# keurfonluu/stochopy

Hardware: AMD Instinct MI355X
Metric: objective-fn evals/sec (higher is better)
Workload: dtype f64; 1 GPU; de_rosenbrock_n128_p4096; method=de, objective=rosenbrock, dim=128, popsize_per_gpu=4096, popsize_total=4096, rng=philox, exchange=none

## Files before the change

include/stochopy_hip.h:

```cpp
#ifndef STOCHOPY_HIP_H
#define STOCHOPY_HIP_H

#include <stdint.h>

#ifdef __cplusplus
extern "C" {
#endif

#define SX_ABI_VERSION 1

enum {
    SX_FUN_ACKLEY = 0,
    SX_FUN_GRIEWANK = 1,
    SX_FUN_QUARTIC = 2,
    SX_FUN_RASTRIGIN = 3,
    SX_FUN_ROSENBROCK = 4,
    SX_FUN_SPHERE = 5,
    SX_FUN_STYBLINSKI_TANG = 6,
    SX_FUN_COUNT = 7
};

enum { SX_DE_RAND1BIN = 0, SX_DE_RAND2BIN = 1, SX_DE_BEST1BIN = 2, SX_DE_BEST2BIN = 3 };

enum {
    SX_RNG_HOST = 0,
    SX_RNG_PHILOX = 1
};

#define SX_STATUS_NONE 100

int sx_abi_version(void);
const char *sx_last_error(void);
int sx_device_count(void);
int sx_struct_size(int which);

int sx_sum_plan(int64_t m, int32_t *out, int cap);
int64_t sx_fun_terms(int fun_id, int n);

int64_t sx_num_partials(int64_t P, int n);
int sx_rows_per_workgroup(int n);
int sx_wide_from(void);
int64_t sx_de_num_partials(int64_t P, int n, int wide_from);
int sx_eval(int fun_id, const double *X, int64_t P, int n, int64_t ldx, const double *xm, const double *xstd,
            double *f, double *part_f, int64_t *part_i, void *stream);

int sx_philox_lhs(double *X, int64_t rows, int n, int64_t ld, int64_t row0, int64_t P, const double *lower,
                  const double *upper, uint32_t key0, uint32_t key1, void *stream);

int sx_argmin(const double *f, int64_t P, double *ws_f, int64_t *ws_i, int64_t ws_len, int64_t *out_idx,
              double *out_val, void *stream);

typedef struct sx_state {
    int64_t it;
    int64_t gbidx;
    double gfit;
    double dx;
    int32_t status;
    int32_t done;
    int64_t reserved[3];
} sx_state;

typedef struct sx_de_args {
    double *buf0, *buf1;
    double *fit;
    double *candfit;
    double *gbest;
    const double *lower;
    const double *upper;
    sx_state *state;
    double *part_f;
    int64_t *part_i;
    const double *r1;
    const int32_t *donors;
    const int32_t *irand;
    const double *resample;
    int64_t P;
    int64_t ld;
    int64_t row0;
    int32_t n;
    int32_t fun_id;
    int32_t strategy;
    int32_t constraints;
    int32_t rng;
    int32_t maxiter;
    int32_t wide_from;
    int32_t pad;
    double F, CR, xtol, ftol;
    uint32_t key0, key1;
} sx_de_args;

int sx_de_generation(const sx_de_args *a, int finalize, void *stream);

int sx_select_finalize(const double *part_f, const int64_t *part_i, int64_t npart, const double *rows0,
                       const double *rows1, int64_t ld, int n, double *gbest, sx_state *state, int maxiter,
                       double xtol, double ftol, void *stream);

int sx_shard_best(const double *part_f, const int64_t *part_i, int64_t npart, const double *rows0,
                  const double *rows1, int64_t ld, int n, const sx_state *state, int64_t row0, double *record,
                  void *stream);
int sx_gather_finalize(const double *records, int world, int n, double *gbest, sx_state *state, int maxiter,
                       double xtol, double ftol, void *stream);
int sx_de_shard_generation(const struct sx_de_args *a, double *record, void *stream);

typedef struct sx_graph sx_graph;
int sx_de_graph_create(const sx_de_args *a, int ngen, sx_graph **out);
int sx_de_chain_launch(const sx_de_args *a, int parity, int finalize_only, void *stream);
int sx_de_chain_graph_create(const sx_de_args *a, int ngen, int start_parity, sx_graph **out);
int sx_graph_launch(sx_graph *g, void *stream);
int sx_graph_destroy(sx_graph *g);

#define SX_MAX_PEERS 8
#define SX_IPC_HANDLE_BYTES 64
typedef struct sx_xchg_args {
    uint64_t *peer[SX_MAX_PEERS];
    int32_t world, rank;
    int64_t timeout_ticks;
    int32_t *error;
    uint64_t *relay;
    const double *pop0[SX_MAX_PEERS];
    const double *pop1[SX_MAX_PEERS];
    int64_t global_rows, shard_rows;
} sx_xchg_args;
int64_t sx_xchg_bytes(int world, int n);
int64_t sx_xchg_relay_bytes(int n);
int sx_xchg_alloc(int64_t bytes, void **ptr, void *handle);
int sx_xchg_free(void *ptr);
int sx_pop_alloc(int64_t bytes, void **ptr, void *handle);
int sx_xchg_open(const void *handle, void **ptr);
int sx_xchg_close(void *ptr);
int sx_xchg_probe(const sx_xchg_args *x, int n, int rounds, void *stream);
int sx_xchg_read_record(const sx_xchg_args *x, int n, int parity, int src, double *record, void *stream);
int sx_xchg_finalize(const double *part_f, const int64_t *part_i, int64_t npart, const double *rows0,
                     const double *rows1, int64_t ld, int n, int64_t row0, double *gbest, sx_state *state, int maxiter,
                     double xtol, double ftol, const sx_xchg_args *x, void *stream);
int sx_de_p2p_launch(const sx_de_args *a, const sx_xchg_args *x, int parity, int finalize_only, void *stream);
int sx_de_p2p_graph_create(const sx_de_args *a, const sx_xchg_args *x, int ngen, int start_parity, sx_graph **out);

typedef struct sx_pso_args {
    double *X, *V, *pbest;
    double *pbestfit;
    double *candfit;
    double *gbest;
    const double *lower;
    const double *upper;
    sx_state *state;
    double *part_f;
    int64_t *part_i;
    const double *r1;
    const double *r2;
    const uint64_t *pending_restart;
    int64_t P;
    int64_t ld;
    int64_t row0;
    int32_t n;
    int32_t fun_id;
    int32_t constraints;
    int32_t rng;
    int32_t maxiter;
    int32_t pad_;
    double w, c1, c2, xtol, ftol;
    uint32_t key0, key1;
} sx_pso_args;

int sx_pso_generation(const sx_pso_args *a, int finalize, void *stream);

int sx_pso_radius(const sx_pso_args *a, double *part_r, void *stream);
int sx_pso_restart_select(const sx_pso_args *a, const double *part_r, double delta, double gamma, uint64_t *out3,
                          void *stream);
int sx_pso_restart_apply(const sx_pso_args *a, const uint64_t *sel3, const int64_t *host_rows, const double *host_x,
                         int64_t host_count, void *stream);
// ... 169 lines not shown
```

stochopy_amd/_lib.py:

```python
import ctypes as C
import os

_HERE = os.path.dirname(os.path.abspath(__file__))
LIB_PATH = os.path.join(_HERE, "lib", "libstochopy_hip.so")

SX_STATUS_NONE = 100
NARROW_DIM, WIDE_DIM = 4096, 262144


def wide_from():
    return int(lib().sx_wide_from())
SX_RNG_HOST, SX_RNG_PHILOX = 0, 1

FUN_IDS = {
    "ackley": 0,
    "griewank": 1,
    "quartic": 2,
    "rastrigin": 3,
    "rosenbrock": 4,
    "sphere": 5,
    "styblinski_tang": 6,
}
DE_STRATEGIES = {"rand1bin": 0, "rand2bin": 1, "best1bin": 2, "best2bin": 3}
DE_DONORS = {"rand1bin": 3, "rand2bin": 5, "best1bin": 2, "best2bin": 4}

vp = C.c_void_p
i64 = C.c_int64
i32 = C.c_int32
f64 = C.c_double


class SxState(C.Structure):
    _fields_ = [("it", i64), ("gbidx", i64), ("gfit", f64), ("dx", f64), ("status", i32), ("done", i32),
                ("reserved", i64 * 3)]


class SxDeArgs(C.Structure):
    _fields_ = [
        ("buf0", vp), ("buf1", vp), ("fit", vp), ("candfit", vp), ("gbest", vp), ("lower", vp),
        ("upper", vp), ("state", vp), ("part_f", vp), ("part_i", vp), ("r1", vp), ("donors", vp),
        ("irand", vp), ("resample", vp),
        ("P", i64), ("ld", i64), ("row0", i64),
        ("n", i32), ("fun_id", i32), ("strategy", i32), ("constraints", i32), ("rng", i32), ("maxiter", i32),
        ("wide_from", i32), ("pad", i32),
        ("F", f64), ("CR", f64), ("xtol", f64), ("ftol", f64),
        ("key0", C.c_uint32), ("key1", C.c_uint32),
    ]


class SxPsoArgs(C.Structure):
    _fields_ = [
        ("X", vp), ("V", vp), ("pbest", vp), ("pbestfit", vp), ("candfit", vp), ("gbest", vp), ("lower", vp),
        ("upper", vp), ("state", vp), ("part_f", vp), ("part_i", vp), ("r1", vp), ("r2", vp), ("pending_restart", vp),
        ("P", i64), ("ld", i64), ("row0", i64),
        ("n", i32), ("fun_id", i32), ("constraints", i32), ("rng", i32), ("maxiter", i32), ("pad", i32),
        ("w", f64), ("c1", f64), ("c2", f64), ("xtol", f64), ("ftol", f64),
        ("key0", C.c_uint32), ("key1", C.c_uint32),
    ]


SX_MAX_PEERS = 8
SX_IPC_HANDLE_BYTES = 64


class SxXchgArgs(C.Structure):
    _fields_ = [("peer", vp * SX_MAX_PEERS), ("world", i32), ("rank", i32), ("timeout_ticks", i64), ("error", vp),
                ("relay", vp), ("pop0", vp * SX_MAX_PEERS), ("pop1", vp * SX_MAX_PEERS), ("global_rows", i64),
                ("shard_rows", i64)]


class SxCmaState(C.Structure):
    _fields_ = [("it", i64), ("nfev", i64), ("best_row", i64), ("fbest", f64), ("sigma", f64), ("sigma_next", f64),
                ("tmp_coef", f64), ("psnorm", f64), ("status", i32), ("done", i32), ("stop_it", i64),
                ("reserved", f64 * 6)]


class SxVdArgs(C.Structure):
    _fields_ = [
        ("Z", vp), ("ary", vp), ("arx", vp), ("fit", vp), ("xmean", vp), ("xold", vp), ("dx", vp), ("dvec", vp),
        ("vvec", vp), ("vn", vp), ("pc", vp), ("zinj", vp), ("dy", vp), ("w", vp), ("mws", vp), ("mout", vp),
        ("besthist", vp), ("xm", vp), ("xstd", vp), ("xbest", vp), ("hist_x", vp), ("hist_f", vp), ("order", vp),
        ("state", vp), ("pen_ws", vp), ("pen_order", vp), ("P", i64), ("hist_rows", i64),
        ("n", i32), ("mu", i32), ("fun_id", i32), ("maxiter", i32), ("ilim", i32), ("pad", i32),
        ("cs", f64), ("ds", f64), ("cc", f64), ("c1", f64), ("cmu", f64), ("mueff", f64), ("wsum", f64), ("xtol", f64),
        ("ftol", f64), ("insigma", f64), ("key0", C.c_uint32), ("key1", C.c_uint32),
    ]


class SxCmaArgs(C.Structure):
    _fields_ = [
        ("Z", vp), ("arx", vp), ("fit", vp), ("xmean", vp), ("xold", vp), ("ps", vp), ("pc", vp), ("C", vp), ("B", vp),
        ("D", vp), ("eigw", vp), ("w", vp), ("Y", vp), ("part", vp), ("step", vp), ("isc", vp), ("xnew", vp),
        ("ypart", vp), ("besthist", vp), ("xm", vp), ("xstd", vp),
        ("xbest", vp), ("hist_x", vp), ("hist_f", vp), ("order", vp), ("state", vp), ("eigh_ws", vp),
        ("pen_ws", vp), ("pen_order", vp),
        ("eigh_ws_bytes", i64), ("P", i64), ("hist_rows", i64),
        ("n", i32), ("mu", i32), ("fun_id", i32), ("maxiter", i32), ("ilim", i32), ("eig_sweeps", i32),
        ("cs", f64), ("cc", f64), ("c1", f64), ("cmu", f64), ("damps", f64), ("chind", f64), ("mueff", f64),
        ("xtol", f64), ("ftol", f64), ("insigma", f64),
        ("key0", C.c_uint32), ("key1", C.c_uint32),
    ]


SX_SAMPLE_MCMC, SX_SAMPLE_HMC = 0, 1
SX_JAC_FINITE_DIFF, SX_JAC_ANALYTIC = 0, 1


class SxSampleArgs(C.Structure):
    _fields_ = [
        ("cur", vp), ("fcur", vp), ("facc", vp), ("fmin", vp), ("xbest", vp),
        ("iacc", vp), ("imin", vp), ("nacc", vp), ("nfeas", vp),
        ("x0", vp), ("xall", vp), ("funall", vp), ("lower", vp), ("upper", vp), ("step", vp), ("normals", vp), ("logu", vp),
        ("C", i64), ("x0_stride", i64), ("maxiter", i64),
        ("n", i32), ("fun_id", i32), ("method", i32), ("rng", i32), ("reject", i32), ("k", i32), ("nleap", i32), ("jac", i32),
        ("fd_step", f64),
        ("key0", C.c_uint32), ("key1", C.c_uint32),
    ]


PROTOTYPES = {
    "sx_abi_version": (C.c_int, []),
    "sx_wide_from": (C.c_int, []),
    "sx_last_error": (C.c_char_p, []),
    "sx_device_count": (C.c_int, []),
    "sx_struct_size": (C.c_int, [C.c_int]),
    "sx_sum_plan": (C.c_int, [i64, vp, C.c_int]),
    "sx_fun_terms": (i64, [C.c_int, C.c_int]),
    "sx_num_partials": (i64, [i64, C.c_int]),
# ... 124 lines not shown
```

stochopy_amd/csrc/sx_de_kernel.hpp:

```cpp
#pragma once
#ifndef SX_DE_XM
#error "define SX_DE_XM (0, 1 or 2) before including sx_de_kernel.hpp"
#endif
#include <type_traits>
#include <vector>

#include "sx_device.hpp"
#include "sx_host.hpp"
#include "sx_rowops.hpp"
#include "sx_xchg.hpp"

namespace sx {
int make_plan_arg(int fun_id, int n, PlanArg *out);
int add_finalize_node(hipGraph_t graph, hipGraphNode_t *prev, const double *part_f, const int64_t *part_i,
                      int64_t npart, const double *rows0, const double *rows1, int64_t ld, int n, double *gbest,
                      sx_state *state, int maxiter, double xtol, double ftol);
int check_xchg_args(const sx_xchg_args *x);
}
using namespace sx;

#if defined(SX_TRACE) && SX_DE_XM == 1
__device__ unsigned long long sx_trace_buf[1024 * 16];
#define SX_TP(k)                                                                              \
    do {                                                                                      \
// ... 89 lines not shown
            uint64_t w[8];
#pragma unroll
            for (int u = 0; u < 8; ++u) {
                const int j = j0 + u * (int)blockDim.x;
                w[u] = j < nwords ? ll_load(src + j) : 0;
            }
#pragma unroll
            for (int u = 0; u < 8; ++u) {
                const int j = j0 + u * (int)blockDim.x;
                if (j >= nwords) continue;
                while (!ll_ok(w[u], tag)) {
                    if ((int64_t)(wall_clock64() - t0) > x.timeout_ticks) {
                        atomicExch(x.error, 1);
                        lost = true;
                        break;
                    }
                    w[u] = ll_load(src + j);
                }
                __hip_atomic_store(dst + j, w[u], __ATOMIC_RELAXED, __HIP_MEMORY_SCOPE_AGENT);
            }
        }
        __builtin_amdgcn_fence(__ATOMIC_RELEASE, "agent");
        __syncthreads();
        if (threadIdx.x == 0)
            __hip_atomic_store(dst + xchg_slot_words(a.n), (uint64_t)tag, __ATOMIC_RELEASE, __HIP_MEMORY_SCOPE_AGENT);
        if (wave != 0) return;
    }
    if (lane == 0) {
        int status = SX_STATUS_NONE;
        if (it >= 2) {
            if (gf <= a.ftol)
                status = 1;
            else if (it >= a.maxiter)
                status = -1;
        }
        sx_state *so = a.state + (mode == 1 ? 2 : 1 - chain_p);
        so->it = it;
        so->gbidx = gi;
        so->gfit = gf;
        so->dx = 0.0;
        so->status = status;
        so->done = status != SX_STATUS_NONE;
        so->reserved[0] = prev_winner;
        so->reserved[1] = winner;
    }
}

constexpr int kStep = 4;

#ifndef SX_DE_NFIX_WAVES
#define SX_DE_NFIX_WAVES 1
#endif
#ifndef SX_DE_WAVE_ROWS_WAVES
#define SX_DE_WAVE_ROWS_WAVES 1
#endif
template <int FUN, int RNG, int XM, int LPR, bool FULL, int NFIX = 0, int STRAT = -1, bool ONEB = false>
__global__ __launch_bounds__(kMaxWavesPerBlock *kWave, (NFIX != 0 && XM <= 1) ? SX_DE_NFIX_WAVES
                                                       : (NFIX == 0 && XM == 0 && STRAT >= 0 && LPR == kWave) ? SX_DE_WAVE_ROWS_WAVES
                                                                                                                 : 1) void de_generation_kernel(const sx_state *const sin_pre,
                                                                                 const double *const pf_pre,
                                                                                 const int64_t *const pi_pre,
                                                                                 const int64_t npart,
                                                                                 const sx_de_args a,
                                                                                 const PlanArg plan,
                                                                                 const int chain_p, const int mode,
                                                                                 const sx_xchg_args x) {
    constexpr bool CHAIN = XM >= 1;
    constexpr bool P2P = XM == 2;
    extern __shared__ __attribute__((aligned(16))) double lds[];
    __shared__ double sf[kMaxRowsPerBlock];
    __shared__ int64_t si[kMaxRowsPerBlock];
    __shared__ double s_gf;
    __shared__ int64_t s_gi;
    __shared__ int s_winner;
    SX_TP(0);
    const int n = NFIX ? NFIX : a.n;
    const int64_t P = a.P, ld = a.ld;
    const RowIds<LPR> id(P, P2P ? 1 : 0);
    const int l = id.l;
    const int64_t rowc = id.rowc;
    double *U = lds + id.slot * gen_row_stride(n);

    const sx_state *sin = (CHAIN && !P2P) ? sin_pre : CHAIN ? a.state + chain_p : a.state;
    constexpr int kRecPerLane = 8;
    double pfv[kRecPerLane];
    using rec_t = typename std::conditional<LPR == kWave, int32_t, int64_t>::type;
    constexpr rec_t kNoRec = LPR == kWave ? (rec_t)INT32_MAX : (rec_t)INT64_MAX;
    rec_t piv[kRecPerLane];
#ifndef SX_CHAIN_REC_WAVE0
#define SX_CHAIN_REC_WAVE0 1
#endif
    if (CHAIN && !P2P && (!SX_CHAIN_REC_WAVE0 || id.wave == 0)) {
        const double *pf = pf_pre;
        const int64_t *pi = pi_pre;
        const int per = (int)((npart + kWave - 1) / kWave);
        const int64_t k0 = (int64_t)id.lane * per;
#pragma unroll
        for (int u = 0; u < kRecPerLane; ++u) {
            const bool in = u < per && k0 + u < npart;
            pfv[u] = in ? pf[k0 + u] : __builtin_huge_val();
            piv[u] = in ? (rec_t)pi[k0 + u] : kNoRec;
        }
    }
    if (P2P && blockIdx.x == 0) {
        p2p_service(a, x, chain_p, mode, npart, sin, LPR == kWave);
        return;
    }
    if (sin->done) {
        if (CHAIN && mode == 1 && threadIdx.x == 0) a.state[2] = *sin;
        return;
    }
    const int64_t it = CHAIN ? sin->it + 1 : sin->it;
    SX_TP(6);

    const uint32_t gen = (uint32_t)(it + 1);
    const double *__restrict__ cur = (it & 1) ? a.buf1 : a.buf0;
    double *__restrict__ nxt = (it & 1) ? a.buf0 : a.buf1;
    const double fold = a.fit[rowc];
    const double *__restrict__ xi = cur + rowc * ld;
    const uint32_t grow = (uint32_t)(a.row0 + rowc);
    const int strategy = STRAT >= 0 ? STRAT : a.strategy;
    const int k = donors_of(strategy);
    const bool repair = STRAT >= 0 ? false : a.constraints != 0;
    const bool use_best = strategy == SX_DE_BEST1BIN || strategy == SX_DE_BEST2BIN;

    int64_t d[kMaxDonors];
    int irand;
    const bool gdon = P2P && x.global_rows > 0;
    if (RNG == SX_RNG_PHILOX) {
        philox_donors(gdon ? x.global_rows : P, k, gdon ? a.row0 + rowc : rowc, grow, gen, a.key0, a.key1, n, d, irand);
    } else {
#pragma unroll
        for (int t = 0; t < kMaxDonors; ++t) d[t] = t < k ? (int64_t)a.donors[(int64_t)t * P + rowc] : 0;
        irand = a.irand[rowc];
    }
    SX_TP(1);
    const double *pd[kMaxDonors];
#pragma unroll
    for (int t = 0; t < kMaxDonors; ++t) pd[t] = cur + d[t] * ld;
    if (gdon) {
#pragma unroll
        for (int t = 0; t < kMaxDonors; ++t) {
            const int owner = (int)(d[t] / x.shard_rows);
            const int64_t lrow = d[t] - (int64_t)owner * x.shard_rows;
            const double *base = nullptr;
#pragma unroll
            for (int r = 0; r < SX_MAX_PEERS; ++r)
                if (r == owner) base = (it & 1) ? x.pop1[r] : x.pop0[r];
            pd[t] = base + lrow * ld;
        }
    }
    const double F = a.F, CR = a.CR;
    const double *r1row = RNG == SX_RNG_HOST ? a.r1 + rowc * (int64_t)n : nullptr;
    const double *rsrow = (RNG == SX_RNG_HOST && repair) ? a.resample + rowc * (int64_t)n : nullptr;

    struct Batch {
        double x[kStep], d[kMaxDonors][kStep], r[kStep], rs[kStep];
    };
    Batch B0;
    auto load_batch = [&](int q0, Batch &bt) {
        double(&bx)[kStep] = bt.x;
        double(&bd)[kMaxDonors][kStep] = bt.d;
        double(&br)[kStep] = bt.r;
        double(&brs)[kStep] = bt.rs;
#pragma unroll
        for (int t = 0; t < kStep; ++t) {
            const int e = (q0 + t) * LPR + l;
            const bool in = FULL || e < n;
            bx[t] = in ? xi[e] : 0.0;
#pragma unroll
            for (int s = 0; s < kMaxDonors; ++s) {
                if (P2P && gdon)
                    bd[s][t] = (s < k && in) ? __hip_atomic_load(pd[s] + e, __ATOMIC_RELAXED, __HIP_MEMORY_SCOPE_SYSTEM)
                                             : 0.0;
                else
                    bd[s][t] = (s < k && in) ? pd[s][e] : 0.0;
            }
            br[t] = 2.0;
            brs[t] = 0.0;
            if (RNG == SX_RNG_HOST && in) {
                br[t] = r1row[e];
                if (repair) brs[t] = rsrow[e];
            }
        }
        if (RNG == SX_RNG_PHILOX) {
#pragma unroll
            for (int t = 0; t < kStep; t += 2) {
                const U4 w = philox4x32_10((uint32_t)((q0 + t) >> 1) * (uint32_t)LPR + (uint32_t)l, grow, gen, kPurposeDeCross,
                                           a.key0, a.key1);
                br[t] = u53(w.x, w.y);
                br[t + 1] = u53(w.z, w.w);
            }
            if (repair) {
#pragma unroll
                for (int t = 0; t < kStep; ++t) {
                    const int e = (q0 + t) * LPR + l;
                    if (FULL || e < n)
                        brs[t] = a.lower[e] + (a.upper[e] - a.lower[e]) *
                                                  philox_u53(e, LPR, grow, gen, kPurposeDeResample, a.key0, a.key1);
                }
            }
// ... 29 lines not shown
            if (id.lane == 0) {
                s_gf = bf;
                s_gi = bi;
                s_winner = ok ? winner : -1;
                if (!ok) atomicExch(x.error, 1);
            }
        }
        __syncthreads();
        const int winner = s_winner;
        if (winner < 0) return;
        const double bf = s_gf;
        const int64_t bi = s_gi;
        if (it >= 2 && (bf <= a.ftol || it >= a.maxiter)) return;
        gbidx = bi;
        gbw = LPR == kWave ? rel + 4 : x.peer[x.rank] + xchg_slot_offset(n, chain_p, winner) + 4;
        part_f_out = a.part_f + (int64_t)(1 - chain_p) * npart;
        part_i_out = a.part_i + (int64_t)(1 - chain_p) * npart;
        if (gdon) load_batch(0, B0);
    } else if (CHAIN) {
        double bf = 0.0;
        int64_t bi = 0;
        if (!SX_CHAIN_REC_WAVE0 || id.wave == 0) {
        double lm[kRecPerLane / 2];
#pragma unroll
        for (int u = 0; u < kRecPerLane / 2; ++u) lm[u] = fmin(pfv[2 * u], pfv[2 * u + 1]);
        const double lmin = fmin(fmin(lm[0], lm[1]), fmin(lm[2], lm[3]));
        bf = wave_min_f64(lmin);
        rec_t br = piv[0];
        double bv = pfv[0];
#pragma unroll
        for (int u = kRecPerLane - 1; u >= 0; --u)
            if (pfv[u] == bf) br = piv[u], bv = pfv[u];
        unsigned long long hit = __ballot(lmin == bf);
        bool lnan = false;
#pragma unroll
        for (int u = 0; u < kRecPerLane; ++u) lnan |= is_nan(pfv[u]);
        const unsigned long long nanl = __ballot(lnan);
        if (nanl) {
            hit = nanl;
#pragma unroll
            for (int u = kRecPerLane - 1; u >= 0; --u)
                if (is_nan(pfv[u])) br = piv[u], bv = pfv[u];
        }
        const int src = hit ? (int)__ffsll((long long)hit) - 1 : 0;
        bf = readlane_f64(bv, src);
        if (LPR == kWave) {
            bi = (int64_t)__builtin_amdgcn_readlane((int)br, src);
        } else {
            const int lo = __builtin_amdgcn_readlane((int)((int64_t)br & 0xffffffffll), src);
            const int hi = __builtin_amdgcn_readlane((int)((int64_t)br >> 32), src);
            bi = ((int64_t)hi << 32) | (int64_t)(unsigned)lo;
        }
        }
        if (SX_CHAIN_REC_WAVE0) {
            if (id.wave == 0 && id.lane == 0) s_gf = bf, s_gi = bi;
            __syncthreads();
            bf = s_gf, bi = s_gi;
        }
        int status = SX_STATUS_NONE;
        if (it >= 2) {
            if (bf <= a.ftol)
                status = 1;
            else if (it >= a.maxiter)
                status = -1;
        }
        if (blockIdx.x == 0 && threadIdx.x == 0) {
            sx_state *so = a.state + (mode == 1 ? 2 : 1 - chain_p);
            so->it = it;
            so->gbidx = bi;
            so->gfit = bf;
            so->dx = 0.0;
            so->status = status;
            so->done = status != SX_STATUS_NONE;
            so->reserved[0] = sin->gbidx;
        }
        if (status != SX_STATUS_NONE || mode == 1) return;
        gbidx = bi;
        part_f_out = a.part_f + (int64_t)(1 - chain_p) * npart;
        part_i_out = a.part_i + (int64_t)(1 - chain_p) * npart;
    } else {
        gbidx = sin->gbidx;
    }
    const double *__restrict__ gb = P2P ? cur : a.gbest != nullptr ? a.gbest : cur + gbidx * ld;

    const int nq = (n + LPR - 1) / LPR;
    constexpr bool kRegRow = NFIX != 0 || LPR < kWave || ONEB;
    double keep[kStep];
    auto trial_batch = [&](int q0, const Batch &bt) {
        const double(&bx)[kStep] = bt.x;
        const double(&bd)[kMaxDonors][kStep] = bt.d;
        const double(&br)[kStep] = bt.r;
        const double(&brs)[kStep] = bt.rs;
        double g[kStep];
        if (P2P) {
            if (use_best) {
                const uint64_t t0 = wall_clock64();
                for (int attempt = 0;; ++attempt) {
                    uint64_t lo[kStep], hi[kStep];
                    bool ok = true;
                    const bool cached = LPR == kWave && attempt == 0;
#pragma unroll
                    for (int t = 0; t < kStep; ++t) {
                        const int e = (q0 + t) * LPR + l;
                        const bool in = FULL || e < n;
                        if (cached) {
                            const ulonglong2 w2 =
                                in ? *reinterpret_cast<const ulonglong2 *>(gbw + 2 * e) : make_ulonglong2(0, 0);
                            lo[t] = w2.x;
                            hi[t] = w2.y;
                        } else if (LPR == kWave) {
                            lo[t] = in ? __hip_atomic_load(gbw + 2 * e, __ATOMIC_RELAXED, __HIP_MEMORY_SCOPE_AGENT) : 0;
                            hi[t] = in ? __hip_atomic_load(gbw + 2 * e + 1, __ATOMIC_RELAXED, __HIP_MEMORY_SCOPE_AGENT) : 0;
                        } else {
                            lo[t] = in ? ll_load(gbw + 2 * e) : 0;
                            hi[t] = in ? ll_load(gbw + 2 * e + 1) : 0;
                        }
                    }
#pragma unroll
                    for (int t = 0; t < kStep; ++t) {
                        const int e = (q0 + t) * LPR + l;
                        if (FULL || e < n) ok = ok && ll_ok(lo[t], xtag) && ll_ok(hi[t], xtag);
                        g[t] = ll_join_f64(lo[t], hi[t]);
                    }
                    if (ok) break;
                    if ((int64_t)(wall_clock64() - t0) > x.timeout_ticks) {
                        atomicExch(x.error, 1);
                        break;
                    }
                }
            } else {
#pragma unroll
                for (int t = 0; t < kStep; ++t) g[t] = 0.0;
            }
        } else {
#pragma unroll
            for (int t = 0; t < kStep; ++t) {
                const int e = (q0 + t) * LPR + l;
                g[t] = (use_best && (FULL || e < n)) ? gb[e] : 0.0;
            }
        }
#pragma unroll
        for (int t = 0; t < kStep; ++t) {
            const int e = (q0 + t) * LPR + l;
            if (FULL || e < n) {
                const double v = de_mutant(strategy, g[t], bd[0][t], bd[1][t], bd[2][t], bd[3][t], bd[4][t], F);
                double cand = (e == irand || br[t] <= CR) ? v : bx[t];
                if (repair && (cand < a.lower[e] || cand > a.upper[e])) cand = brs[t];
                U[e] = cand;
                if (kRegRow) keep[t] = cand;
            }
        }
    };
    if constexpr (LPR < kWave) {
        trial_batch(0, B0);
    } else {
        trial_batch(0, B0);
        if constexpr (!ONEB) {
            for (int q0 = kStep; q0 < nq; q0 += kStep) {
                load_batch(q0, B0);
                trial_batch(q0, B0);
            }
        }
    }

    SX_TP(2);
    const double fc = row_objective<FUN, LPR, FULL, NFIX, SX_LONG_STATIC, ONEB>(U, n, plan, l);
    SX_TP(3);
    const bool better = fc < fold;
    if (FULL || id.active) {
        double *__restrict__ xo = nxt + id.row * ld;
        if constexpr (kRegRow) {
#pragma unroll
            for (int t = 0; t < kStep; ++t)
                if (NFIX != 0 || l + t * LPR < n) st_stream(xo + l + t * LPR, better ? keep[t] : B0.x[t]);
        } else {
            const double *__restrict__ src = better ? U : xi;
            for (int e0 = l; e0 < n; e0 += kStep * LPR) {
                double v[kStep];
#pragma unroll
                for (int t = 0; t < kStep; ++t) v[t] = (FULL || e0 + t * LPR < n) ? src[e0 + t * LPR] : 0.0;
#pragma unroll
                for (int t = 0; t < kStep; ++t)
                    if (FULL || e0 + t * LPR < n) xo[e0 + t * LPR] = v[t];
            }
        }
        if (l == 0) {
            if (better) a.fit[id.row] = fc;
            if (a.candfit != nullptr) a.candfit[id.row] = fc;
        }
    }
    SX_TP(4);
    block_partial<LPR>(better ? fc : fold, id, sf, si, part_f_out, part_i_out);
    SX_TP(5);
}

typedef void (*de_kernel_t)(const sx_state *, const double *, const int64_t *, const int64_t, const sx_de_args,
                            const PlanArg, const int, const int, const sx_xchg_args);

template <int RNG, int XM, int LPR, bool FULL, int NFIX = 0, int STRAT = -1, bool ONEB = false>
de_kernel_t pick_kernel_lpr(int fun_id) {
    constexpr bool SPECIAL = STRAT != -1 || ONEB || NFIX != 0;
    switch (fun_id) {
        case SX_FUN_ACKLEY: return de_generation_kernel<SX_FUN_ACKLEY, RNG, XM, LPR, FULL, NFIX, STRAT, ONEB>;
        case SX_FUN_RASTRIGIN: return de_generation_kernel<SX_FUN_RASTRIGIN, RNG, XM, LPR, FULL, NFIX, STRAT, ONEB>;
        case SX_FUN_ROSENBROCK: return de_generation_kernel<SX_FUN_ROSENBROCK, RNG, XM, LPR, FULL, NFIX, STRAT, ONEB>;
        case SX_FUN_SPHERE: return de_generation_kernel<SX_FUN_SPHERE, RNG, XM, LPR, FULL, NFIX, STRAT, ONEB>;
    }
    if constexpr (!SPECIAL) {
        switch (fun_id) {
            case SX_FUN_GRIEWANK: return de_generation_kernel<SX_FUN_GRIEWANK, RNG, XM, LPR, FULL, NFIX, STRAT, ONEB>;
            case SX_FUN_QUARTIC: return de_generation_kernel<SX_FUN_QUARTIC, RNG, XM, LPR, FULL, NFIX, STRAT, ONEB>;
            case SX_FUN_STYBLINSKI_TANG: return de_generation_kernel<SX_FUN_STYBLINSKI_TANG, RNG, XM, LPR, FULL, NFIX, STRAT, ONEB>;
        }
    }
    return nullptr;
}

template <int RNG, int XM, int LPR, bool FULL, int NFIX>
de_kernel_t pick_kernel_fixed(int fun_id, int strategy, int constraints) {
    if constexpr (XM == 2 && LPR != 32) {
        return pick_kernel_lpr<RNG, XM, LPR, FULL, NFIX>(fun_id);
    } else {
        if (constraints != 0 || !hot_objective(fun_id)) return pick_kernel_lpr<RNG, XM, LPR, FULL, NFIX>(fun_id);
        switch (strategy) {
            case SX_DE_RAND1BIN: return pick_kernel_lpr<RNG, XM, LPR, FULL, NFIX, NFIX ? SX_DE_RAND1BIN : -1>(fun_id);
            case SX_DE_BEST1BIN: return pick_kernel_lpr<RNG, XM, LPR, FULL, NFIX, NFIX ? SX_DE_BEST1BIN : -1>(fun_id);
        }
        return pick_kernel_lpr<RNG, XM, LPR, FULL, NFIX>(fun_id);
    }
}

template <int RNG, int XM, int LPR>
de_kernel_t pick_kernel_general(int fun_id, int strategy, int constraints, int n) {
    if constexpr (XM <= 1 && RNG == SX_RNG_PHILOX) {
        if (!hot_objective(fun_id)) return pick_kernel_lpr<RNG, XM, LPR, false>(fun_id);
        if constexpr (LPR == kWave) {
            if (n <= 4 * kWave && constraints == 0 && strategy == SX_DE_BEST1BIN)
                return pick_kernel_lpr<RNG, XM, LPR, false, 0, SX_DE_BEST1BIN, true>(fun_id);
            if (n <= 4 * kWave && constraints == 0 && strategy == SX_DE_RAND1BIN)
                return pick_kernel_lpr<RNG, XM, LPR, false, 0, SX_DE_RAND1BIN, true>(fun_id);
        }
        if (constraints == 0 && strategy == SX_DE_BEST1BIN) return pick_kernel_lpr<RNG, XM, LPR, false, 0, SX_DE_BEST1BIN>(fun_id);
        if (constraints == 0 && strategy == SX_DE_RAND1BIN) return pick_kernel_lpr<RNG, XM, LPR, false, 0, SX_DE_RAND1BIN>(fun_id);
    }
    return pick_kernel_lpr<RNG, XM, LPR, false>(fun_id);
}

template <int RNG, int XM>
de_kernel_t pick_kernel(int fun_id, int n, int64_t P, int strategy, int constraints) {
    constexpr bool CH = XM >= 1;
    const int lpr = lanes_per_row(n);
    const bool full = CH && n % (kStep * lpr) == 0 && P % rows_per_block(n) == 0;
    constexpr bool FX = CH && RNG == SX_RNG_PHILOX;
    const bool fix = FX && full && n == kStep * lpr && hot_objective(fun_id);
    switch (lpr) {
        case 16:
            if (fix) return pick_kernel_fixed<RNG, XM, 16, CH, FX ? kStep * 16 : 0>(fun_id, strategy, constraints);
            return full ? pick_kernel_lpr<RNG, XM, 16, CH>(fun_id) : pick_kernel_general<RNG, XM, 16>(fun_id, strategy, constraints, n);
        case 32:
            if (fix) return pick_kernel_fixed<RNG, XM, 32, CH, FX ? kStep * 32 : 0>(fun_id, strategy, constraints);
            return full ? pick_kernel_lpr<RNG, XM, 32, CH>(fun_id) : pick_kernel_general<RNG, XM, 32>(fun_id, strategy, constraints, n);
    }
    if (fix) return pick_kernel_fixed<RNG, XM, 64, CH, FX ? kStep * 64 : 0>(fun_id, strategy, constraints);
    return full ? pick_kernel_lpr<RNG, XM, 64, CH>(fun_id) : pick_kernel_general<RNG, XM, 64>(fun_id, strategy, constraints, n);
}

}
```

stochopy_amd/optimize/_de.py:

```python
import ctypes as C
import os
import warnings

import numpy as np

from .. import _device, _lib, _rng
from . import _common
from ._helpers import register
from ._population import _PopulationRun

__all__ = ["minimize"]


def minimize(
    fun,
    bounds,
    x0=None,
    args=(),
    maxiter=100,
    popsize=10,
    mutation=0.5,
    recombination=0.9,
    strategy="best1bin",
    seed=None,
# ... 224 lines not shown
            ngen -= self.GRAPH_CHUNK
        for _ in range(ngen):
            _lib.check(ctx.L.sx_de_generation(C.byref(self.args), 1, ctx.stream_ptr), "sx_de_generation")

    def _setup(self):
        ctx, P, n = self.ctx, self.P, self.n
        t = _device.torch()
        self.stream = _rng.make_init_stream(self.rng, self.seed)
        d_bounds = ctx.upload_async(np.concatenate([self.lower, self.upper]))
        self.d_lower, self.d_upper = d_bounds[:n], d_bounds[n:]
        if self.global_donors:
            self.bufs = list(self.px.share_population(P, n, self.Ptotal))
        else:
            self.bufs = [ctx.empty((P, n)), ctx.empty((P, n))]
        if self.x0 is None and self.rng == "philox":
            _rng.philox_latin_hypercube(ctx, self.bufs[1], self.row0, self.Ptotal, self.d_lower, self.d_upper, self.seed)
        else:
            if self.x0 is not None:
                X0 = np.array(self.x0, dtype=np.float64)
            else:
                X0 = self.stream.latin_hypercube(self.Ptotal, n, self.lower, self.upper)
            if self.world is not None:
                X0 = np.ascontiguousarray(X0[self.row0 : self.row0 + P])
            self.bufs[1].copy_(ctx.upload(X0))
        self.fit = ctx.empty((P,))
        self.candfit = ctx.empty((P,))
        npart = self.npart
        self.part_f = ctx.empty((npart,))
        self.part_i = ctx.empty((npart,), dtype=t.int64)
        _common.evaluate_rows(ctx, self.fun_id, self.bufs[1], n, self.fit)
        self.candfit.copy_(self.fit)
        quiet_start = (self.chain and self.world is None and self.px is None and self.callback is None
                       and not self.return_all and self.external is None)
        if quiet_start:
            rec_f = t.full((2, npart), float("inf"), dtype=t.float64, device=ctx.device)
            rec_i = t.full((2, npart), np.iinfo(np.int64).max, dtype=t.int64, device=ctx.device)
            _lib.check(ctx.L.sx_argmin(_device.ptr(self.fit), P, _device.ptr(self.part_f), _device.ptr(self.part_i),
                                       npart, _device.ptr(rec_i), _device.ptr(rec_f), ctx.stream_ptr), "sx_argmin")
            g, gfit0 = 0, 0.0
            self.gbest = None
        else:
            out_i = ctx.empty((1,), dtype=t.int64)
            out_f = ctx.empty((1,))
            _lib.check(ctx.L.sx_argmin(_device.ptr(self.fit), P, _device.ptr(self.part_f), _device.ptr(self.part_i),
                                       npart, _device.ptr(out_i), _device.ptr(out_f), ctx.stream_ptr), "sx_argmin")
            g = int(out_i.cpu()[0])
            gfit0 = float(out_f.cpu()[0])
            self.gbest = self.bufs[1][g].clone()
        if self.world is not None and self.px is None:
            from ..parallel import best_of_records

            self.record = ctx.empty((n + 2,))
            self.records = ctx.empty((self.world.size, n + 2))
            self.record[0] = gfit0
            self.record[1] = float(self.row0 + g)
            self.record[2:].copy_(self.gbest)
            self.world.all_gather_records(self.record, self.records)
            wbest, gfit0, g = best_of_records(self.records.cpu().numpy())
            self.gbest.copy_(self.records[wbest, 2:])
        st = _lib.SxState(it=1, gbidx=g, gfit=gfit0, dx=0.0, status=_lib.SX_STATUS_NONE, done=0)
        if self.chain:
            s0 = _lib.SxState(it=0, gbidx=g, gfit=gfit0, dx=0.0, status=_lib.SX_STATUS_NONE, done=0)
            raw = np.frombuffer(bytes(s0) + bytes(st) + bytes(st), dtype=np.int64).copy()
            self.state = ctx.upload_async(raw)
            if quiet_start:
                self.part_f, self.part_i = rec_f, rec_i
            else:
                pf = np.full((2, npart), np.inf)
                pi = np.full((2, npart), np.iinfo(np.int64).max, dtype=np.int64)
                pf[0, 0], pi[0, 0] = gfit0, g
                self.part_f = ctx.upload(pf)
                self.part_i = ctx.upload(pi)
        else:
            self.state = ctx.upload(np.frombuffer(bytes(st), dtype=np.int64).copy())
        key0, key1 = _rng.philox_key(self.seed) if self.rng == "philox" else (0, 0)
        a = _lib.SxDeArgs()
        a.buf0, a.buf1 = self.bufs[0].data_ptr(), self.bufs[1].data_ptr()
        if self.immediate:
            a.buf0 = a.buf1
        a.fit, a.candfit = self.fit.data_ptr(), self.candfit.data_ptr()
        a.lower, a.upper, a.state = self.d_lower.data_ptr(), self.d_upper.data_ptr(), self.state.data_ptr()
        a.part_f, a.part_i = self.part_f.data_ptr(), self.part_i.data_ptr()
        a.gbest = None if self.chain else self.gbest.data_ptr()
        a.P, a.ld, a.row0, a.n = P, n, self.row0, n
        a.wide_from = self.wide_from
        a.fun_id, a.strategy = (self.fun_id if self.external is None else 0), _lib.DE_STRATEGIES[self.strategy]
        if self.external is not None:
            self.cand = ctx.empty((P, n))
            self.cand_f = ctx.empty((P,))
        self.it_enq = 1
        a.constraints = 1 if self.constraints == "Random" else 0
        a.rng = _lib.SX_RNG_PHILOX if self.rng == "philox" else _lib.SX_RNG_HOST
        a.maxiter = self.maxiter
        a.F, a.CR, a.xtol, a.ftol = self.F, self.CR, self.xtol, self.ftol
        a.key0, a.key1 = key0, key1
        self.args = a
        if self.rng == "numpy-legacy":
            self.h_r1 = t.empty((P, n), dtype=t.float64).pin_memory()
            self.h_don = t.empty((self.k, P), dtype=t.int32).pin_memory()
            self.h_irand = t.empty((P,), dtype=t.int32).pin_memory()
            self.d_r1 = ctx.empty((P, n))
            self.d_don = ctx.empty((self.k, P), dtype=t.int32)
            self.d_irand = ctx.empty((P,), dtype=t.int32)
            a.r1, a.donors, a.irand = self.d_r1.data_ptr(), self.d_don.data_ptr(), self.d_irand.data_ptr()
            if a.constraints:
                self.h_rs = t.empty((P, n), dtype=t.float64).pin_memory()
                self.d_rs = ctx.empty((P, n))
                a.resample = self.d_rs.data_ptr()
        self.st = st
        if self.world is not None and (self.return_all or self.callback is not None):
            self.Xfull = ctx.empty((self.Ptotal, n))
            self.candfull = ctx.empty((self.Ptotal,))
            if self.px is not None:
                st = self.read_state()
                self.gbest.copy_(ctx.upload(self._best_row(st)))
        if self.return_all:
            self.nout = int(np.ceil(self.verbosity * self.Ptotal))
            rows = max(self.nout, 1)
            self.xall = ctx.empty((self.maxiter, rows, n))
            self.funall = ctx.empty((self.maxiter, rows))
            if self.nout > 0:
                X1, f1 = self._whole_population(1)
                self.xall[0].copy_(X1[: self.nout])
                self.funall[0].copy_(f1[: self.nout])
            else:
                self.xall[0, 0].copy_(self.gbest if self.world is not None else self.bufs[1][g])
                self.funall[0, 0] = st.gfit
        self.st = st

    def _population(self, it):
        return self.bufs[1] if self.immediate else self.bufs[it & 1]

    def _best_row(self, st):
        if self.px is not None:
            return self.px.read_record((st.it - 1) & 1, int(st.reserved[1]))[2]
        if self.chain:
            return self._population(st.it)[st.gbidx].cpu().numpy()
        return self.gbest.cpu().numpy()

    def _settle_status(self, st):
        status = int(st.status)
        if self.chain and status == 1:
            if self.px is not None:
                prev = self.px.read_record(st.it & 1, int(st.reserved[0]))[2]
            else:
                prev = self._population(st.it - 1)[st.reserved[0]].cpu().numpy()
            if np.linalg.norm(prev - self._best_row(st)) <= self.xtol:
                status = 0
        return status

    def _host_draws(self):
        s = self.stream
        s.random(None, out=self.h_r1.numpy())
        if self.immediate:
            rs = self.h_rs.numpy() if self.args.constraints else None
            s.de_async_draws(self.P, self.k, self.n, self.h_don.numpy(), self.h_irand.numpy(), self.lower, self.upper, rs)
            self.d_r1.copy_(self.h_r1, non_blocking=True)
            self.d_don.copy_(self.h_don, non_blocking=True)
            self.d_irand.copy_(self.h_irand, non_blocking=True)
            if rs is not None:
                self.d_rs.copy_(self.h_rs, non_blocking=True)
            return
        s.de_donors(self.P, self.k, out=self.h_don.numpy())
        self.h_irand.numpy()[:] = s.randint(self.n, self.P)
        self.d_r1.copy_(self.h_r1, non_blocking=True)
        self.d_don.copy_(self.h_don, non_blocking=True)
# ... 103 lines not shown
```

Before: 605.4 million evals/s.

## Skip rewriting unchanged DE rows using a per-row win flag

Adds a per-row byte flag recording whether a row's trial won in the previous generation. With ping-pong buffers, a row that lost in both the previous and the current generation already holds the correct value in the next buffer, so its write-back is skipped. This cuts global store traffic when most trials are rejected. The change also vectorizes the partial-record loads for common slice sizes, prefetches the first batch of best-vector elements ahead of the trial loop, and reads the state fields once. In exchange it adds a flag read and a conditional flag write per row. The flag is only enabled for single-GPU, non-immediate, non-external, non-wide runs.

```diff
diff --git a/include/stochopy_hip.h b/include/stochopy_hip.h
--- a/include/stochopy_hip.h
+++ b/include/stochopy_hip.h
@@ -86,6 +86,7 @@
     int32_t wide_from;
     int32_t pad;
     double F, CR, xtol, ftol;
+    uint8_t *rowflag;
     uint32_t key0, key1;
 } sx_de_args;
 
diff --git a/stochopy_amd/_lib.py b/stochopy_amd/_lib.py
--- a/stochopy_amd/_lib.py
+++ b/stochopy_amd/_lib.py
@@ -44,6 +44,7 @@
         ("n", i32), ("fun_id", i32), ("strategy", i32), ("constraints", i32), ("rng", i32), ("maxiter", i32),
         ("wide_from", i32), ("pad", i32),
         ("F", f64), ("CR", f64), ("xtol", f64), ("ftol", f64),
+        ("rowflag", vp),
         ("key0", C.c_uint32), ("key1", C.c_uint32),
     ]
 
diff --git a/stochopy_amd/csrc/sx_de_kernel.hpp b/stochopy_amd/csrc/sx_de_kernel.hpp
--- a/stochopy_amd/csrc/sx_de_kernel.hpp
+++ b/stochopy_amd/csrc/sx_de_kernel.hpp
@@ -195,6 +195,8 @@
     double *U = lds + id.slot * gen_row_stride(n);
 
     const sx_state *sin = (CHAIN && !P2P) ? sin_pre : CHAIN ? a.state + chain_p : a.state;
+    const int done0 = sin->done;
+    const int64_t it0 = sin->it;
     constexpr int kRecPerLane = 8;
     double pfv[kRecPerLane];
     using rec_t = typename std::conditional<LPR == kWave, int32_t, int64_t>::type;
@@ -208,28 +210,60 @@
         const int64_t *pi = pi_pre;
         const int per = (int)((npart + kWave - 1) / kWave);
         const int64_t k0 = (int64_t)id.lane * per;
-#pragma unroll
-        for (int u = 0; u < kRecPerLane; ++u) {
-            const bool in = u < per && k0 + u < npart;
-            pfv[u] = in ? pf[k0 + u] : __builtin_huge_val();
-            piv[u] = in ? (rec_t)pi[k0 + u] : kNoRec;
+        auto load_slices = [&](auto per_c) {
+            constexpr int PER = decltype(per_c)::value;
+            const double *f = pf + (int64_t)id.lane * PER;
+            const int64_t *r = pi + (int64_t)id.lane * PER;
+            if constexpr (PER == 1) {
+                pfv[0] = f[0];
+                piv[0] = (rec_t)r[0];
+            } else {
+#pragma unroll
+                for (int u = 0; u < PER; u += 2) {
+                    const double2 fv = *reinterpret_cast<const double2 *>(f + u);
+                    const longlong2 rv = *reinterpret_cast<const longlong2 *>(r + u);
+                    pfv[u] = fv.x, pfv[u + 1] = fv.y;
+                    piv[u] = (rec_t)rv.x, piv[u + 1] = (rec_t)rv.y;
+                }
+            }
+#pragma unroll
+            for (int u = PER; u < kRecPerLane; ++u) pfv[u] = __builtin_huge_val(), piv[u] = kNoRec;
+        };
+        const bool whole = npart == (int64_t)per * kWave && (((uintptr_t)pf | (uintptr_t)pi) & 15) == 0;
+        if (whole && per == 4) {
+            load_slices(std::integral_constant<int, 4>());
+        } else if (whole && per == 8) {
+            load_slices(std::integral_constant<int, 8>());
+        } else if (whole && per == 2) {
+            load_slices(std::integral_constant<int, 2>());
+        } else if (whole && per == 1) {
+            load_slices(std::integral_constant<int, 1>());
+        } else {
+#pragma unroll
+            for (int u = 0; u < kRecPerLane; ++u) {
+                const bool in = u < per && k0 + u < npart;
+                pfv[u] = in ? pf[k0 + u] : __builtin_huge_val();
+                piv[u] = in ? (rec_t)pi[k0 + u] : kNoRec;
+            }
         }
     }
     if (P2P && blockIdx.x == 0) {
         p2p_service(a, x, chain_p, mode, npart, sin, LPR == kWave);
         return;
     }
-    if (sin->done) {
+    if (done0) {
         if (CHAIN && mode == 1 && threadIdx.x == 0) a.state[2] = *sin;
         return;
     }
-    const int64_t it = CHAIN ? sin->it + 1 : sin->it;
+    const int64_t it = CHAIN ? it0 + 1 : it0;
     SX_TP(6);
 
     const uint32_t gen = (uint32_t)(it + 1);
     const double *__restrict__ cur = (it & 1) ? a.buf1 : a.buf0;
     double *__restrict__ nxt = (it & 1) ? a.buf0 : a.buf1;
     const double fold = a.fit[rowc];
+    const uint8_t *flagp = a.rowflag != nullptr ? a.rowflag + rowc : reinterpret_cast<const uint8_t *>(a.fit + rowc);
+    const bool won_prev = (*flagp != 0) | (a.rowflag == nullptr);
     const double *__restrict__ xi = cur + rowc * ld;
     const uint32_t grow = (uint32_t)(a.row0 + rowc);
     const int strategy = STRAT >= 0 ? STRAT : a.strategy;
@@ -425,11 +459,21 @@
         gbidx = sin->gbidx;
     }
     const double *__restrict__ gb = P2P ? cur : a.gbest != nullptr ? a.gbest : cur + gbidx * ld;
+    double gfirst[kStep];
+    if constexpr (!P2P) {
+#pragma unroll
+        for (int t = 0; t < kStep; ++t) {
+            const int e = t * LPR + l;
+            gfirst[t] = (use_best && (FULL || e < n)) ? gb[e] : 0.0;
+        }
+        __builtin_amdgcn_sched_barrier(0);
+    }
 
     const int nq = (n + LPR - 1) / LPR;
     constexpr bool kRegRow = NFIX != 0 || LPR < kWave || ONEB;
     double keep[kStep];
-    auto trial_batch = [&](int q0, const Batch &bt) {
+    auto trial_batch = [&](int q0, const Batch &bt, auto first_c) {
+        constexpr bool FIRST = decltype(first_c)::value;
         const double(&bx)[kStep] = bt.x;
         const double(&bd)[kMaxDonors][kStep] = bt.d;
         const double(&br)[kStep] = bt.r;
@@ -475,6 +519,9 @@
 #pragma unroll
                 for (int t = 0; t < kStep; ++t) g[t] = 0.0;
             }
+        } else if constexpr (FIRST) {
+#pragma unroll
+            for (int t = 0; t < kStep; ++t) g[t] = gfirst[t];
         } else {
 #pragma unroll
             for (int t = 0; t < kStep; ++t) {
@@ -495,13 +542,13 @@
         }
     };
     if constexpr (LPR < kWave) {
-        trial_batch(0, B0);
+        trial_batch(0, B0, std::true_type());
     } else {
-        trial_batch(0, B0);
+        trial_batch(0, B0, std::true_type());
         if constexpr (!ONEB) {
             for (int q0 = kStep; q0 < nq; q0 += kStep) {
                 load_batch(q0, B0);
-                trial_batch(q0, B0);
+                trial_batch(q0, B0, std::false_type());
             }
         }
     }
@@ -510,7 +557,7 @@
     const double fc = row_objective<FUN, LPR, FULL, NFIX, SX_LONG_STATIC, ONEB>(U, n, plan, l);
     SX_TP(3);
     const bool better = fc < fold;
-    if (FULL || id.active) {
+    if ((FULL || id.active) && (better || won_prev)) {
         double *__restrict__ xo = nxt + id.row * ld;
         if constexpr (kRegRow) {
 #pragma unroll
@@ -527,10 +574,11 @@
                     if (FULL || e0 + t * LPR < n) xo[e0 + t * LPR] = v[t];
             }
         }
-        if (l == 0) {
-            if (better) a.fit[id.row] = fc;
-            if (a.candfit != nullptr) a.candfit[id.row] = fc;
-        }
+    }
+    if ((FULL || id.active) && l == 0) {
+        if (better) a.fit[id.row] = fc;
+        if (a.candfit != nullptr) a.candfit[id.row] = fc;
+        if (a.rowflag != nullptr && better != won_prev) a.rowflag[id.row] = better ? 1 : 0;
     }
     SX_TP(4);
     block_partial<LPR>(better ? fc : fold, id, sf, si, part_f_out, part_i_out);
diff --git a/stochopy_amd/optimize/_de.py b/stochopy_amd/optimize/_de.py
--- a/stochopy_amd/optimize/_de.py
+++ b/stochopy_amd/optimize/_de.py
@@ -330,6 +330,10 @@
         a.lower, a.upper, a.state = self.d_lower.data_ptr(), self.d_upper.data_ptr(), self.state.data_ptr()
         a.part_f, a.part_i = self.part_f.data_ptr(), self.part_i.data_ptr()
         a.gbest = None if self.chain else self.gbest.data_ptr()
+        self.rowflag = None
+        if self.world is None and not self.immediate and self.external is None and not self.wide:
+            self.rowflag = t.ones((P,), dtype=t.uint8, device=ctx.device)
+            a.rowflag = self.rowflag.data_ptr()
         a.P, a.ld, a.row0, a.n = P, n, self.row0, n
         a.wide_from = self.wide_from
         a.fun_id, a.strategy = (self.fun_id if self.external is None else 0), _lib.DE_STRATEGIES[self.strategy]
```

After: 607.9 million evals/s, median of 6. No clear change (+0.4%).
